# rwl/blu

Hardware: AMD Instinct MI355X
Metric: factorize nnz/s + achieved HBM GB/s, 100k x 100k 10-nnz/col basis (higher is better)
Workload: dtype f64

## Files before the change

### blu_amd/csrc/blu_dev.h

```cpp
#pragma once
#include <hip/hip_runtime.h>
#include <stdint.h>
#include <hip/hip_cooperative_groups.h>
#include <rocprim/warp/warp_reduce.hpp>
#include <rocprim/warp/warp_scan.hpp>

#define BLU_WAVE 64

#ifndef BLU_DYN_SHARED
#define BLU_DYN_SHARED(T, name, bytes) extern __shared__ __attribute__((aligned(16))) T name[]
#endif
#ifdef BLU_PROFILE_FILLS
#define FILL_STAMP_BEGIN() long long fill_t0_ = (long long)__builtin_amdgcn_s_memtime()
#define FILL_STAMP(S, k)                                                 \
    do {                                                                 \
        if (threadIdx.x == 0) {                                          \
            const long long t_ = (long long)__builtin_amdgcn_s_memtime(); \
            (S)->prof[k] += t_ - fill_t0_;                               \
            fill_t0_ = t_;                                               \
        }                                                                \
    } while (0)
#else
#define FILL_STAMP_BEGIN() \
    do {                   \
    } while (0)
#define FILL_STAMP(S, k) \
    do {                 \
    } while (0)
#endif
#ifdef BLU_EMU_BUILD
#define BLU_WAVES_PER_EU(lo, hi)
#else
#define BLU_WAVES_PER_EU(lo, hi) __attribute__((amdgpu_waves_per_eu(lo, hi)))
#endif

enum {
    ST_RUNNING = 0,
    ST_DONE = 1,
    ST_STOPPED = 2,
    ST_NEED_L = 3,
    ST_NEED_U = 4,
    ST_NEED_CW = 5,
    ST_NEED_RW = 6,
    ST_INVALID_ARG = 7,
    ST_ERROR = 8
};

struct Scalars {
    int status;
    int err_line;
    int rank;
    int rankdef;
    int rank0;
    int min_colnz;
    int min_rownz;
    int pivot_row;
    int pivot_col;
    int bump_size;
    int cused, rused;
    int lused, uused;
    int need;
    int l_nz, u_nz;
    int fill_paths;
    long long matrix_nz;
    long long bump_nz;
    long long nsearch_pivot;
    long long factor_flops;
    long long nexpand;
    long long ngarbage;
    long long d3_hits;
    long long npivot_kind[6];
    long long nfast[4];
    long long nrun[4];
    double min_pivot, max_pivot;
    double onenorm, infnorm;
    double norm_l, norm_u, normest_l_inv, normest_u_inv, condest_l, condest_u, residual_test;
    long long prof[48];
    long long prof2[14];
};

#define DEVLU_SCALARS(X)                                                                               \
    X(int, m)                                                                                          \
    X(int, nzbias)                                                                      \
    X(int, maxsearch)                                                                                  \
    X(int, pad)                                                                                        \
    X(int, search_rows)                                                                                \
    X(int, no_fast)                    \
    X(int, skip_stats)              \
    X(double, droptol)                                                                                 \
    X(double, abstol)                                                                                  \
    X(double, reltol)                                                                                  \
    X(double, stretch)                                                                                 \
    X(long long, b_i_len)                                                                              \
    X(int, nzcap)                                                                                      \
    X(int, carena_cap)                                                                                 \
    X(int, rarena_cap)                                                                                 \
    X(int, lcap)                                                                                       \
    X(int, ucap)

#define DEVLU_ARRAYS_HOT(X)                                                                            \
    X(int, pinv) X(int, qinv) X(int, prow) X(int, pcol)                                                \
    X(LineRec, crec) X(LineRec, rrec) X(HeadRec, chead) X(HeadRec, rhead)                              \
    X(int, cidx) X(double, cval) X(int, ridx)                                                          \
    X(int, lbeg) X(int, ubeg) X(int, lidx) X(int, uidx) X(double, lval) X(double, uval)
#define DEVLU_ARRAYS_COLD(X)                                                                           \
    X(const unsigned long long, b_begin) X(const unsigned long long, b_end) X(const unsigned long long, b_i) \
    X(const double, b_x)                                                                               \
    X(int, bc_ptr) X(int, bc_idx) X(double, bc_val) X(int, bt_ptr) X(int, bt_idx) X(double, bt_val)    \
    X(int, rowmark) X(int, colmark) X(int, tnew) X(int, tnewr) X(double, txrj)                         \
    X(unsigned long long, tmask) X(double, gwork) X(int, iw0) X(int, iw1) X(int, iw2)
#define DEVLU_ARRAYS(X) DEVLU_ARRAYS_HOT(X) DEVLU_ARRAYS_COLD(X)

struct __attribute__((aligned(32))) LineRec {
    int beg, len, cap;
    int flink, blink;
    int spare;
    double max;
};
struct __attribute__((aligned(8))) HeadRec {
    int flink, blink;
};
static_assert(sizeof(LineRec) == 32 && sizeof(HeadRec) == 8, "record layout");
#define LINEREC_BEG 0
#define LINEREC_LEN 4
#define LINEREC_CAP 8
#define LINEREC_FLINK 12
#define LINEREC_BLINK 16
#define LINEREC_MAX 24

struct DevLU {
#define X(T, n) T n;
// ... 477 lines not shown
```

### blu_amd/csrc/blu_hip.hip

```cpp
#include <hip/hip_runtime.h>

#include <algorithm>
#include <cmath>
#include <cstdio>
#include <cstdlib>
#include <cstring>
#include <string>
#include <vector>

#include "../../include/blu_hip.h"
#include "blu_dev.h"
#include "k_finish.hip"
#define BLU_NS pv_single
#define BLU_CFG_WAVE 0
#include "k_pivot.hip"
#undef BLU_NS
#undef BLU_CFG_WAVE
#define BLU_NS pv_wave
#define BLU_CFG_WAVE 1
#include "k_pivot.hip"
#undef BLU_NS
#undef BLU_CFG_WAVE
#define BLU_NS pv_wave2
#define BLU_CFG_WAVE 2
// ... 473 lines not shown
    case BLU_STAT_TIME_FACTORIZE: return h->t_total;
    case BLU_STAT_TIME_SINGLETONS: return h->t_phase[0];
    case BLU_STAT_TIME_SEARCH_PIVOT: {
        double tot = 0.0;
        for (int k = 0; k < 4; k++) tot += (double)s.prof[k];
        return tot > 0.0 ? h->t_pivot * (double)s.prof[0] / tot : 0.0;
    }
    case BLU_STAT_TIME_ELIM_PIVOT: {
        double tot = 0.0;
        for (int k = 0; k < 4; k++) tot += (double)s.prof[k];
        return tot > 0.0 ? h->t_pivot * (1.0 - (double)s.prof[0] / tot) : h->t_pivot;
    }
    case BLU_STAT_UPDATE_COST_DENOM: return h->update_cost_denom;
    case BLU_STAT_RANKDEF: return (double)s.rankdef;
    case BLU_STAT_L_MEM: return (double)h->D.lcap;
    case BLU_STAT_U_MEM: return (double)h->D.ucap;
    case BLU_STAT_W_MEM: return (double)h->D.carena_cap + (double)h->D.rarena_cap;
    case BLU_STAT_L_FLOPS: return (double)h->sp_l_flops;
    case BLU_STAT_U_FLOPS: return (double)h->sp_u_flops;
    case BLU_STAT_NFORREST: return h->upd_for_nfact == h->nfactorize ? (double)h->ust.nforrest : 0.0;
    case BLU_STAT_PIVOT_ERROR: return h->upd_for_nfact == h->nfactorize ? h->ust.pivot_error : 0.0;
    case BLU_STAT_R_NZ: return h->upd_for_nfact == h->nfactorize ? (double)h->ust.r_nz : 0.0;
    case BLU_STAT_R_FLOPS: return h->upd_for_nfact == h->nfactorize ? (double)h->ust.r_flops : 0.0;
    case BLU_STAT_MAX_ETA: return h->upd_for_nfact == h->nfactorize ? h->ust.max_eta : 0.0;
    case BLU_STAT_NSYMPERM_TOTAL: return (double)h->ust.nsymperm_total;
    case BLU_STAT_NFORREST_TOTAL: return (double)h->ust.nforrest_total;
    case BLU_STAT_DEV_NUNSYMPERM_TOTAL: return (double)h->ust.nunsymperm_total;
    case BLU_STAT_UPDATE_COST:
        return (h->upd_for_nfact == h->nfactorize ? h->ust.update_cost_numer : 0.0) / blu_hip_get_stat(h, BLU_STAT_UPDATE_COST_DENOM);
    case 44: case 45: case 46: case 47: return h->t_phase[key - 44];
    case 108: case 109: return h->t_phase[key - 108 + 4];
    case 43: return (double)h->sp_branch;
    case BLU_STAT_DEV_TIME_PIVOT_LOOP: return h->t_pivot;
    case BLU_STAT_DEV_TIME_TOTAL: return h->t_total;
    case BLU_STAT_DEV_RELAUNCHES: return (double)h->relaunches;
    case 50: return (double)s.d3_hits;
    case 51: return (double)s.npivot_kind[0];
    case 52: return (double)s.npivot_kind[1];
    case 53: return (double)s.npivot_kind[2];
    case 54: return (double)s.npivot_kind[3];
    case 55: return (double)s.npivot_kind[4];
    case 56: return (double)s.npivot_kind[5];
    case 110: case 111: case 116: case 117: return (double)s.nfast[key < 116 ? key - 110 : key - 114];
    case 112: return (double)s.cused;
    case 113: return (double)s.rused;
    case 114: return (double)h->D.carena_cap;
    case 115: return (double)h->D.lcap;
    case 120: return (double)h->last_pivot_regs;
    case 118: return (double)h->last_pivot_kernel;
    case 119: return (double)s.fill_paths;
    case 121: case 122: return (double)s.nrun[key - 121];
    case 123: return (double)s.nrun[2];
    case 125: return (double)s.nrun[3];
    case 126: return (double)h->chain_defects;
    case 131: case 132: case 133: case 134: case 135: case 136: case 137: case 138: case 139: case 140: case 141: case 142: case 143: case 144:
        return (double)s.prof2[key - 131];
    case 57: return (double)s.err_line;
    case 58: return (double)s.status;
    case 60: case 61: case 62: case 63: case 64: case 65: case 66: case 67: case 68: case 69: case 70: case 71: case 72: case 73: case 74: case 75:
    case 76: case 77: case 78: case 79: case 80: case 81: case 82: case 83:
    case 84: case 85: case 86: case 87: case 88: case 89: case 90: case 91:
    case 92: case 93: case 94: case 95: case 96: case 97: case 98: case 99: case 100: case 101: case 102: case 103: case 104: case 105: case 106: case 107:
        return (double)s.prof[key - 60];
    default: return NAN;
    }
}

extern "C" const char *blu_hip_last_error(const blu_hip *h) { return h ? h->err.c_str() : "null handle"; }
extern "C" const char *blu_hip_version(void)
{
#if defined(BLU_EWCHECK)
    return "blu_hip 0.2 (gfx950; self-checking build: early / speculative searches verified in the kernel)";
#elif defined(BLU_PROFILE)
    return "blu_hip 0.2 (gfx950; phase-timing build)";
#else
    return "blu_hip 0.2 (gfx950)";
#endif
}
extern "C" int blu_hip_device_count(void)
{
    int n = 0;
    if (hipGetDeviceCount(&n) != hipSuccess) return 0;
    return n;
}

static bool ensure_gwork(blu_hip *h, int cols)
{
    if (cols <= h->gwork_cols) return true;
    DevLU &D = h->D;
    const size_t n = (size_t)cols * ((size_t)h->m + 1);
    dfree(D.gwork);
    h->gwork_cols = 0;
    if (!dalloc(h, &D.gwork, n) || !hip_ok(h, hipMemset(D.gwork, 0, n * sizeof(double)), "hipMemset")) return false;
    h->gwork_cols = cols;
    return true;
}
static int64_t grown(blu_hip *h, int64_t cap, int64_t need_extra)
{
    const double f = std::max(1.0, h->realloc_factor);
    int64_t n = (int64_t)((double)(cap + need_extra) * f) + 64;
    return std::min<int64_t>(n, kIntMax);
}
static bool grow_l(blu_hip *h, int need)
{
    DevLU &D = h->D;
    const int64_t n = grown(h, D.lcap, need);
    if (n <= D.lcap) { h->err = "L storage limit (2^31 entries) reached"; return false; }
    if (!dgrow(h, &D.lidx, (size_t)h->hs.lused, (size_t)n) || !dgrow(h, &D.lval, (size_t)h->hs.lused, (size_t)n)) return false;
// ... 597 lines not shown
```

### blu_amd/csrc/k_pivot.hip

```cpp
#include "blu_dev.h"

namespace BLU_NS {

__shared__ int g_pivot_err;
__shared__ int g_pivot_err_line;
#undef DEV_CHECK
#define DEV_CHECK(S, cond)                               \
    do {                                                 \
        if (!(cond)) {                                   \
            set_error((S), ST_ERROR, __LINE__);          \
            g_pivot_err = 1;                             \
        }                                                \
    } while (0)

#if BLU_CFG_WAVE
#include "k_pivot_wave_types.h"
#else
#include "k_pivot_fast_types.h"
#endif

#ifdef BLU_PROFILE
__shared__ long long g_pstamp[56];
#define PROF_STAMP(k)                                                      \
    do {                                                                   \
        if (threadIdx.x == 0) g_pstamp[k] = (long long)__builtin_amdgcn_s_memtime(); \
    } while (0)
#define PROF_STAMP_L0(k)                                                           \
    do {                                                                           \
        if (lane_id() == 0) g_pstamp[k] = (long long)__builtin_amdgcn_s_memtime(); \
    } while (0)
#define PROF_WAIT() asm volatile("s_waitcnt vmcnt(0)" ::: "memory")
#else
#define PROF_STAMP(k) \
    do {              \
    } while (0)
#define PROF_STAMP_L0(k) \
    do {                 \
    } while (0)
#define PROF_WAIT() \
    do {            \
    } while (0)
#endif

struct alignas(16) Sm {
    Fast fa;
    struct alignas(16) {
        int pr, pc, exit_code, head_exit;
    };
    struct alignas(16) {
        int nzc, nzr, pcb, prb;
    };
#ifdef BLU_PROFILE
    long long prof[48];
    long long prof2[14];
#else
    long long prof[1];
#endif
#if !BLU_CFG_WAVE
    Fast fb;
    struct alignas(16) {
        int nx_pr, nx_pc, nx_nzr, nx_where;
    };
    struct alignas(16) {
        int nx_nzc, nx_kind, nx_pcb, nx_prb;
    };
    int nx_nsr, nx_minc;
    int nx_whole;
    int mg;
    long long nrun[4];
#endif
    int rank, rankdef, min_colnz, min_rownz;
    int cused, rused, lused, uused;
    int need;
    int flag_small;
    int other_row, where, ncancel, nfill;
    int stop_at, need_search;
    double pivot, other_value;
    long long nsearch, flops, nexpand, d3;
    long long kinds[6];
    long long nfast[4];
    int sh[40];
    long long shl[20];
#if BLU_CFG_WAVE
    unsigned long long wmax[BLU_CFG_WAVE];
#else
    unsigned long long wmax[16];
#endif
#if BLU_CFG_WAVE
    double swork[WV_WCAP];
#else
    double swork[16 * 64];
#endif
};

__device__ __forceinline__ void list_remove1(const LinkF &flink, const LinkB &blink, int e)
{
    const int f = flink[e], b = blink[e];
    flink[b] = f;
    blink[f] = b;
    flink[e] = e;
    blink[e] = e;
}
__device__ __forceinline__ void list_add1(int e, int list, const LinkF &flink, const LinkB &blink, int nelem)
{
    const int t = blink[nelem + list];
    blink[nelem + list] = e;
    blink[e] = t;
    flink[t] = e;
    flink[e] = nelem + list;
}

__device__ __forceinline__ int wave_list_move_batch(const LinkF &flink, const LinkB &blink, int nelem, gcint_p elems, gcint_p keys, int n,
                                                    gint_p mark, int big)
{
    const int lane = lane_id();
    int minkey = big;
    for (int c0 = 0; c0 < n; c0 += 64) {
        const int q = c0 + lane;
        if (q < n && keys[q] >= 0) mark[elems[q]] = 1;
    }
    wave_mem_sync();
    for (int c0 = 0; c0 < n; c0 += 64) {
// ... 982 lines not shown
    if (pc < 0 || pr < 0) return;
    sm->pcb = D.cbeg[pc];
    sm->prb = D.rbeg[pr];
    sm->nzc = D.clen[pc];
    sm->nzr = D.rlen[pr];
    sm->flag_small = 0;
    sm->ncancel = 0;
    DEV_CHECK(S, D.pinv[pr] == -1 && D.qinv[pc] == -1);
    DEV_CHECK(S, sm->nzc >= 1 && sm->nzr >= 1);
    if (sm->lused + (sm->nzc - 1) > D.lcap) {
        sm->exit_code = ST_NEED_L;
        sm->need = sm->nzc - 1;
    } else if (sm->uused + (sm->nzr - 1) > D.ucap) {
        sm->exit_code = ST_NEED_U;
        sm->need = sm->nzr - 1;
    }
}

#if BLU_CFG_WAVE
#include "k_pivot_wave.hip"
#else
__device__ __forceinline__ void pivot_loop_body(DevLU *Ds, int stop_at, Sm *sm, Mc *mc)
{
    const DevGP D(&Ds[blockIdx.x]);
    Scalars *S = D.s;
    const int tid = threadIdx.x, w = wave_id(), lane = lane_id();
    const int m = D.m;

    if (S->status != ST_RUNNING) return;
    if (tid == 0) {
        sm->rank = S->rank;
        sm->rankdef = S->rankdef;
        sm->min_colnz = S->min_colnz;
        sm->min_rownz = S->min_rownz;
        sm->cused = S->cused;
        sm->rused = S->rused;
        sm->lused = S->lused;
        sm->uused = S->uused;
        sm->pr = S->pivot_row;
        sm->pc = S->pivot_col;
        sm->exit_code = 0;
        sm->need = 0;
        sm->nsearch = 0;
        sm->flops = 0;
        sm->nexpand = 0;
        sm->d3 = 0;
        sm->stop_at = stop_at;
        sm->fa.kind = 0;
        sm->fa.ewValid = 0;
        sm->fa.spOk = 0;
        for (int k = 0; k < 6; k++) sm->kinds[k] = 0;
        sm->mg = 0;
        sm->nrun[0] = sm->nrun[1] = sm->nrun[2] = sm->nrun[3] = 0;
#ifdef BLU_PROFILE
        for (int k = 0; k < 48; k++) sm->prof[k] = 0;
        for (int k = 0; k < 14; k++) sm->prof2[k] = 0;
        for (int k = 0; k < 56; k++) g_pstamp[k] = 0;
#endif
    }
    for (int k = tid; k < (int)blockDim.x; k += blockDim.x) sm->swork[k] = 0.0;
    if (tid < 16) sm->wmax[tid] = 0ull;
    for (int k = tid; k < 2 * KGMAX; k += blockDim.x) sm->fa.kg[0][k] = 0ull;
    if (tid == 0) {
        g_pivot_err = 0;
        g_pivot_err_line = 0;
    }
    mc_reset(D, mc, tid, (int)blockDim.x);
    __syncthreads();

#ifdef BLU_PROFILE
#define PROF_ADD(k, a, b)                                                                                           \
    do {                                                                                                            \
        const long long d_ = g_pstamp[a] - g_pstamp[b];                                                             \
        if (g_pstamp[b] >= g_pstamp[0] && d_ >= 0 && d_ < (1LL << 28)) sm->prof[k] += d_;                            \
    } while (0)
#define PROF_ADD2(k, a, b)                                                                                          \
    do {                                                                                                            \
        const long long d_ = g_pstamp[a] - g_pstamp[b];                                                             \
        if (g_pstamp[b] >= g_pstamp[0] && d_ >= 0 && d_ < (1LL << 28)) sm->prof2[k] += d_;                           \
    } while (0)
    auto prof_account = [&](int kind_done, int nzc_done, int nzr_done) {
        {
            const int kk = kind_done == 1 ? 1 : (kind_done == 2 ? 2 : 3);
            PROF_ADD(0, 1, 0);
            PROF_ADD(kk, 2, 1);
            sm->prof[3 + kk] += 1;
            if (kk == 1) {
                const int by = g_pstamp[1] == g_pstamp[0] ? 8 : 11;
                PROF_ADD2(by, 2, 0);
                PROF_ADD2(by + 1, 2, 3);
                sm->prof2[by + 2] += 1;
                PROF_ADD(7, 3, 1);
                PROF_ADD(22, 6, 3);
                PROF_ADD(23, 24, 3);
                PROF_ADD(24, 25, 3);
                PROF_ADD(25, 26, 25);
                PROF_ADD(26, 27, 26);
                PROF_ADD(27, 28, 27);
                PROF_ADD(30, 30, 27);
                PROF_ADD(31, 31, 30);
                PROF_ADD(28, 29, 28);
                PROF_ADD(29, 2, 29);
                sm->prof[32] += nzr_done - 1;
                sm->prof[33] += nzc_done - 1;
                PROF_ADD(34, 33, 1);
                PROF_ADD(35, 34, 33);
                PROF_ADD(36, 35, 34);
                PROF_ADD(37, 36, 35);
                PROF_ADD(38, 37, 36);
                PROF_ADD(39, 38, 37);
                PROF_ADD(40, 3, 38);
                if (g_pstamp[44] > g_pstamp[1]) {
                    PROF_ADD(41, 41, 1);
                    PROF_ADD(42, 42, 41);
                    PROF_ADD(43, 43, 42);
                    PROF_ADD(44, 44, 43);
                    sm->prof[45] += 1;
                }
                if (g_pstamp[46] > g_pstamp[3]) {
                    PROF_ADD(46, 45, 3);
                    PROF_ADD(47, 46, 3);
                    sm->prof2[7] += 1;
                }
            }
            if (kk == 2) {
                PROF_ADD2(0, 1, 0);
                PROF_ADD2(1, 49, 48);
                PROF_ADD2(2, 50, 48);
                PROF_ADD2(3, 51, 48);
                PROF_ADD2(4, 2, 48);
                PROF_ADD2(5, 48, 1);
            }
            if (kk != 3) {
                PROF_ADD(8, 8, 0);
                PROF_ADD(9, 9, 8);
                PROF_ADD(10, 10, 9);
                PROF_ADD(11, 11, 10);
                PROF_ADD(12, 12, 11);
                PROF_ADD(13, 13, 12);
                PROF_ADD(14, 14, 13);
                PROF_ADD(15, 1, 14);
                if (g_pstamp[16] > g_pstamp[8]) {
                    PROF_ADD(16, 17, 16);
                    PROF_ADD(17, 18, 17);
                    PROF_ADD(18, 10, 18);
                    PROF_ADD(19, 19, 8);
                    PROF_ADD(20, 20, 19);
                    sm->prof[21] += 1;
                }
            }
        }
    };
#endif
    long long ew_mcb = 0;
    int ew_fb = 0;
    for (;;) {
        if (w == 0) {
            if (lane == 0) {
                if (g_pivot_err) sm->exit_code = ST_ERROR;
                else if (sm->rank + sm->rankdef >= m) sm->exit_code = ST_DONE;
                else if (sm->stop_at >= 0 && sm->pc < 0 && sm->rank + sm->rankdef >= sm->stop_at) sm->exit_code = ST_STOPPED;
                sm->need_search = sm->pc < 0;
                sm->head_exit = sm->exit_code;
            }
            wave_mem_sync();
            const bool heads_stale = mc->dirty;
            WAVE_LOCKSTEP();
            if (heads_stale) {
                mc_reset(D, mc, lane, 64);
                wave_mem_sync();
            }
            PROF_STAMP(0);
            if (!sm->head_exit) {
                bool handled = false;
                if (sm->need_search) {
// ... 91 lines not shown
        } else {
            if (tid == 0) mc->dirty = 1;
            if (nz_row == 1) ok = pivot_singleton_row(D, sm);
            else if (nz_col == 1) ok = pivot_singleton_col(D, sm);
            else if (nz_col == 2) ok = pivot_doubleton_col(D, sm);
            else ok = pivot_general(D, sm, nz_col - 1 <= 64);
        }
        if (!ok) break;
        PROF_STAMP(2);
#ifdef BLU_PROFILE
        if (tid == 0) prof_account(kind, nz_col, nz_row);
#endif

        if (tid == 0) {
            const int rank = sm->rank;
            if (sm->flag_small && nz_row > 1) {
                for (int pos = D.ubeg[rank]; pos < D.ubeg[rank + 1]; pos++) {
                    const int j = D.uidx[pos];
                    if (D.colmax[j] == 0.0 || D.colmax[j] < D.abstol) {
                        remove_col_serial(D, sm, j);
                        mc->dirty = 1;
                    }
                }
            }
            sm->flops += (long long)(nz_col - 1) * (long long)(nz_row - 1);
            D.pinv[pr] = rank;
            D.qinv[pc] = rank;
            D.prow[rank] = pr;
            D.pcol[rank] = pc;
            sm->pc = -1;
            sm->pr = -1;
            sm->rank = rank + 1;
        }
    }

    if (tid == 0) {
        S->rank = sm->rank;
        S->rankdef = sm->rankdef;
        S->min_colnz = sm->min_colnz;
        S->min_rownz = sm->min_rownz;
        S->cused = sm->cused;
        S->rused = sm->rused;
        S->lused = sm->lused;
        S->uused = sm->uused;
        S->pivot_row = sm->pr;
        S->pivot_col = sm->pc;
        S->need = sm->need;
        S->nsearch_pivot += sm->nsearch;
        S->factor_flops += sm->flops;
        S->nexpand += sm->nexpand;
        S->d3_hits += sm->d3;
        for (int k = 0; k < 6; k++) S->npivot_kind[k] += sm->kinds[k];
        for (int k = 0; k < 4; k++) S->nrun[k] += sm->nrun[k];
#ifdef BLU_PROFILE
        for (int k = 0; k < 48; k++) S->prof[k] += sm->prof[k];
        for (int k = 0; k < 14; k++) S->prof2[k] += sm->prof2[k];
#endif
        if (sm->exit_code == ST_ERROR && g_pivot_err_line) set_error(S, ST_ERROR, g_pivot_err_line);
        if (S->status == ST_RUNNING) S->status = sm->exit_code;
    }
}

__global__ void __launch_bounds__(1024) k_pivot_loop(DevLU *Ds, int stop_at)
{
    __shared__ Sm smem;
    __shared__ Mc mcache;
    pivot_loop_body(Ds, stop_at, &smem, &mcache);
}
#endif

}
#undef PROF_STAMP
#undef PROF_STAMP_L0
#undef PROF_WAIT
#undef COLD
#undef DEV_CHECK
#define DEV_CHECK(S, cond)                                   \
    do {                                                     \
        if (!(cond)) set_error((S), ST_ERROR, __LINE__);     \
    } while (0)
```

### blu_amd/csrc/k_pivot_fast.hip

```cpp

__device__ __forceinline__ unsigned hslot(int k, int bits) { return ((unsigned)k * 2654435761u) >> (32 - bits); }
__device__ __forceinline__ void probe_overrun(int line)
{
    g_pivot_err = 1;
    g_pivot_err_line = line;
}
__device__ __forceinline__ void hrow_insert(Fast *f, int k, int v)
{
    unsigned s = hslot(k, HROW_BITS);
    const unsigned long long want = ((unsigned long long)(unsigned)k << 32) | (unsigned)v;
    for (int n = 0; n < HROW; n++) {
        const unsigned long long old = atomicCAS(&f->hRow[s], ~0ull, want);
        if (old == ~0ull || (int)(old >> 32) == k) return;
        s = (s + 1) & (HROW - 1);
    }
    probe_overrun(__LINE__);
}
__device__ __forceinline__ int hrow_lookup(const Fast *f, int k)
{
    unsigned s = hslot(k, HROW_BITS);
    for (int n = 0; n < HROW; n++) {
        const unsigned long long x = f->hRow[s];
        if ((int)(x >> 32) == k) return (int)(x & 0xffffffffull);
        if (x == ~0ull) return 0;
// ... 1404 lines not shown
    while (ncand < K && nz <= m && !bad) {
        const int k = nz + lane;
        const int h = k <= m ? LC.fl(m + k) : m + k;
        unsigned long long ne = __ballot(k <= m && h != m + k);
        while (ne && ncand < K && !bad) {
            const int b = __ffsll((long long)ne) - 1;
            ne &= ne - 1;
            int j = wave_bcast_i(h, b);
            const int znz = nz + b;
            int guard = 0;
            while (j < m && ncand < K) {
                const int fl = D.cflink.el(j), cb = D.cbeg[j], cl = D.clen[j];
                const double cmx = D.colmax[j];
                if (cl != znz || cmx == 0.0 || !(cmx >= D.abstol) || ++guard > m + 2) {
                    bad = true;
                    break;
                }
                if (lane == 0) {
                    fa->cJ[ncand] = j;
                    fa->cNz[ncand] = znz;
                    fa->cB[ncand] = cb;
                    fa->cL[ncand] = cl;
                    fa->cMx[ncand] = cmx;
                    fa->cOff[ncand] = total;
                }
                total += cl;
                ncand++;
                lastnz = znz;
                j = fl;
            }
        }
        nz += 64;
    }
    if (bad || ncand < K || total > STGMAX) return;
    SPEC_STAT(1);
    if (lane == 0) {
        fa->cOff[ncand] = total;
        fa->ncand = ncand;
        fa->spLastNz = lastnz;
        fa->spOk = 1;
    }
    wave_mem_sync();
    PROF_STAMP_L0(42);
}

__device__ __forceinline__ bool spec_cond(const Sm *sm, const Fast *cs, const int *keys, int n)
{
    const int lane = lane_id();
    if (!sm->fa.spOk || sm->flag_small || cs->anycancel || n >= 64) return false;
    const int kq = lane < n ? keys[lane] : 0x7fffffff;
    return __ballot(kq <= 0) == 0ull;
}

__device__ __forceinline__ void spec_finish(const DevGP &D, Sm *sm, const Fast *cs, int n)
{
    const int lane = lane_id();
    Fast *fa = &sm->fa;
    const int ncand = fa->ncand;
    {
        const int lastnz = fa->spLastNz;
        const int key = lane < n ? cs->tNew[1 + lane] : 0x7fffffff;
        const unsigned long long inb = __ballot(key < lastnz);
        if (inb) {
            int uJ = 0, uNz = 0x7fffffff, uB = 0, uL = 0;
            double uMx = 0.0;
            if (lane < ncand) {
                uJ = fa->cJ[lane];
                uNz = fa->cNz[lane];
                uB = fa->cB[lane];
                uL = fa->cL[lane];
                uMx = fa->cMx[lane];
            }
            int ule = 0;
            for (int i = 0; i < ncand; i++) ule += fa->cNz[i] <= key;
            int before = 0, below = 0;
            unsigned long long mb = inb;
            while (mb) {
                const int b = __ffsll((long long)mb) - 1;
                mb &= mb - 1;
                const int kb = __builtin_amdgcn_readlane(key, b);
                before += (kb < key) || (kb == key && b < lane);
                below += kb < uNz;
            }
            const int posM = ule + before, posU = lane + below;
            wave_mem_sync();
            if (lane < ncand && posU < ncand) {
                fa->cJ[posU] = uJ;
                fa->cNz[posU] = uNz;
                fa->cB[posU] = uB;
                fa->cL[posU] = uL;
                fa->cMx[posU] = uMx;
            }
            if (((inb >> lane) & 1ull) && posM < ncand) {
                fa->cJ[posM] = cs->tJ[1 + lane];
                fa->cNz[posM] = key;
                fa->cB[posM] = cs->tB[1 + lane];
                fa->cL[posM] = key;
                fa->cMx[posM] = cs->tMx[1 + lane];
            }
            wave_mem_sync();
            if (lane == 0) {
                int off = 0;
                for (int i = 0; i < ncand; i++) {
                    fa->cOff[i] = off;
                    off += fa->cL[i];
                }
                fa->cOff[ncand] = off;
            }
            wave_mem_sync();
            SPEC_STAT(4);
        }
    }
    const int total = fa->cOff[ncand];
    if (total > STGMAX) return;
    const int off1 = ncand > 1 ? fa->cOff[1] : 0x7fffffff, off2 = ncand > 2 ? fa->cOff[2] : 0x7fffffff,
              off3 = ncand > 3 ? fa->cOff[3] : 0x7fffffff;
    const long long BIG = 0x7fffffffffffffffLL;
    long long mcb = BIG;
    int fb = 0x7fffffff;
    for (int base = 0; base < total; base += 64) {
        const int f = base + lane;
        if (f < total) {
            const int c = (f >= off1) + (f >= off2) + (f >= off3);
            const int pos = fa->cB[c] + (f - fa->cOff[c]);
            const int idx = D.cidx[pos];
            const double val = D.cval[pos];
            const int rb = D.rbeg[idx], rl = D.rlen[idx], rc = D.rcap[idx];
            fa->sI[f] = idx;
            fa->sV[f] = val;
            fa->sB[f] = rb;
            fa->sL[f] = rl;
            fa->sC[f] = rc;
            const double tol = fmax(D.abstol, D.reltol * fa->cMx[c]);
            const double x = fabs(val);
            if (!(x == 0.0 || x < tol)) {
                const long long cost = (long long)(fa->cNz[c] - 1) * (long long)(rl - 1);
                if (cost < mcb) {
                    mcb = cost;
                    fb = f;
                }
            }
        }
    }
    PROF_WAIT();
    PROF_STAMP_L0(43);
    SPEC_STAT(2);
    const long long key = wave_min_ll(mcb != BIG ? mcb * 256LL + (long long)fb : BIG);
    if (key == BIG) return;
    SPEC_STAT(3);
    if (lane == 0) {
        fa->spKey = key;
        fa->ewNsr = ncand;
        fa->ewValid = 2;
    }
    wave_mem_sync();
    PROF_STAMP_L0(44);
}

__device__ __forceinline__ bool scol_setup_next(const DevGP &D, Sm *sm, Mc *mc, Fast *nxt, int rl_cur);
__device__ __forceinline__ bool small_setup_next(const DevGP &D, Sm *sm, Mc *mc, Fast *nxt, int cnz1_cur, int rnz1_cur);
__device__ __forceinline__ void fast_small(const DevGP &D, Sm *sm, Mc *mc, Fast *fa, int pr, int pc, int nzc, int nzr, long long &ew_mcb, int &ew_fb)
{
    const int w = wave_id(), nw = num_waves(), lane = lane_id();
    const int m = D.m;
    const int cnz1 = nzc - 1, rnz1 = nzr - 1;
    const double pivot = fa->pcV[0];
    DEV_CHECK(D.s, pivot != 0.0);

    double *work = &sm->swork[w * 64];
    const int ntask = rnz1 + cnz1;
    PROF_STAMP(4);
    const bool split = nw >= 8 && rnz1 < 64;
    const int nwt = split ? nw - 1 : nw;
    const LinksC LC{D, mc};
    const bool early = split && !D.search_rows;
    if (split && w == nw - 1) {
        if (early) __builtin_amdgcn_s_setprio(3);
        const bool lnk = fa->tLnk != 0;
        wave_list_unlink_set(LC, fa->tJ + 1, rnz1, -1, InHCol{fa, 1, 0}, pc, lnk ? fa->tFl + 1 : nullptr, lnk ? fa->tBl + 1 : nullptr, -1);
        if (early) {
            wave_mem_sync();
            spec_walk(D, sm, mc);
            __builtin_amdgcn_s_setprio(0);
        }
    }
    for (int base = 0; base < ntask && w < nwt; base += 3 * nwt) {
        int li[3], tt[3];
        double lv[3];
        tt[0] = base + w;
        tt[1] = base + 2 * nwt - 1 - w;
        tt[2] = base + 2 * nwt + w;
        int lb[3], ll[3];
        bool isc[3];
#pragma unroll
        for (int u = 0; u < 3; u++) {
            const int t = tt[u];
            isc[u] = t < rnz1;
            const bool isr = !isc[u] && t < ntask;
            const int q = isc[u] ? t + 1 : 0, p = isr ? t - rnz1 + 1 : 0;
            const int cb_ = fa->tB[q], cl_ = fa->tL[q], rb_ = fa->prB[p], rl_ = fa->prL[p];
            lb[u] = isc[u] ? cb_ : rb_;
            ll[u] = isc[u] ? cl_ : (isr ? rl_ : 0);
        }
#pragma unroll
        for (int u = 0; u < 3; u++) {
            li[u] = -1;
            lv[u] = 0.0;
            if (lane < ll[u]) {
                if (isc[u]) {
                    li[u] = D.cidx[lb[u] + lane];
                    lv[u] = D.cval[lb[u] + lane];
                } else {
                    li[u] = D.ridx[lb[u] + lane];
                }
            }
        }
#ifdef BLU_PROFILE
        if (w == 1 && base == 0) {
            PROF_STAMP_L0(33);
            PROF_WAIT();
            PROF_STAMP_L0(34);
        }
#endif
#pragma unroll
        for (int u = 0; u < 3; u++) {
            const int t = tt[u];
            if (t < rnz1) {
                if (ll[u] <= 64) fast_col_short(D, sm, mc, fa, t + 1, work, li[u], lv[u], pr, cnz1, pivot);
                else fast_col(D, sm, mc, fa, t + 1, work, li[u], lv[u], pr, cnz1, pivot);
            } else if (t < ntask) {
                if (ll[u] <= 64) fast_row_short(D, sm, fa, t - rnz1 + 1, li[u], pc, rnz1);
                else fast_row(D, sm, fa, t - rnz1 + 1, li[u], pc, rnz1);
            }
#ifdef BLU_PROFILE
            if (w == 1 && base == 0) PROF_STAMP_L0(35 + u);
#endif
        }
    }
#ifdef BLU_PROFILE
    if (w == 1) {
        PROF_WAIT();
        PROF_STAMP_L0(38);
    }
#endif
    PROF_STAMP(5);
    __syncthreads();
    PROF_STAMP(3);
    if (fa->anycancel) {
        for (int p = 1 + w; p <= cnz1; p += nw) fast_fixrow(D, fa, p, rnz1);
        __syncthreads();
    }
    const bool spec = early && (w == 0 || w == nw - 1) && spec_cond(sm, fa, fa->tNew + 1, rnz1);
    Fast *other = fa == &sm->fa ? &sm->fb : &sm->fa;
    if (w == 0 && !spec) {
        bool merged = false;
        if (early) {
            early_search(D, sm, mc, fa, fa->tJ + 1, fa->tNew + 1, fa->tB + 1, fa->tMx + 1, rnz1, 1, ew_mcb, ew_fb);
            merged = scol_setup_next(D, sm, mc, other, rnz1 + 1);
        }
        if (lane == 0) sm->mg = merged ? 1 : 0;
    }
    if (w == nw - 1 && spec) {
        spec_finish(D, sm, fa, rnz1);
        PROF_STAMP_L0(45);
        const bool merged = small_setup_next(D, sm, mc, other, cnz1, rnz1);
        if (lane == 0) sm->mg = merged ? 1 : 0;
        PROF_STAMP_L0(46);
    }
    if (w == (early ? 3 : 0)) {
        fast_write_u(D, sm, fa, 1, rnz1, -1);
        if (lane == 0) {
            D.colmax[pc] = fa->pcV[0];
            D.clen[pc] = 0;
            D.rlen[pr] = 0;
            sm->kinds[3]++;
        }
        PROF_STAMP_L0(6);
    }
    if (w == 1 % nw) {
        fast_write_l(D, sm, fa, cnz1);
        PROF_STAMP_L0(24);
    }
    if (w == 2 % nw) {
        PROF_STAMP_L0(25);
        const int mn = split ? wave_list_append_set(LC, m, fa->tJ + 1, fa->tNew + 1, rnz1, m + 2, sm->fa.kg[0], mc->pFl + 1)
                             : wave_list_move_batch_set(LC, m, fa->tJ + 1, fa->tNew + 1, rnz1, InHCol{fa, 1, 0}, m + 2, pc, sm->fa.kg[0]);
        if (lane == 0 && mn < sm->min_colnz) sm->min_colnz = mn;
        if (lane == 0) {
            mc->prevValid = split && fa == &sm->fa ? 1 : 0;
            mc->prevBase = 1;
        }
        PROF_WAIT();
        PROF_STAMP_L0(29);
    }
    if (D.search_rows && w == 3 % nw) {
        if (lane == 0) list_remove1(D.rflink, D.rblink, pr);
        wave_mem_sync();
        const int mn = wave_list_move_batch_set(LinksG{D.rflink, D.rblink}, m, fa->pcI + 1, fa->rNew + 1, cnz1, InHRow{fa}, m + 2, -1, sm->fa.kg[1]);
        if (lane == 0 && mn < sm->min_rownz) sm->min_rownz = mn;
    }
    __syncthreads();
}

__device__ __forceinline__ bool scol_setup_next(const DevGP &D, Sm *sm, Mc *mc, Fast *nxt, int rl_cur)
{
    const int lane = lane_id();
    Fast *st = &sm->fa;
    if (st->ewValid != 1) return false;
    if (g_pivot_err || mc->dirty) return false;
    const int nrd = sm->rank + 1 + sm->rankdef;
    if (nrd >= D.m || (sm->stop_at >= 0 && nrd >= sm->stop_at)) return false;
    const int pc = st->cJ[0], pr = st->sI[0], prb = st->sB[0], nzr = st->sL[0];
    if (nzr < 2 || nzr >= 64) return false;
    if (sm->lused > D.lcap || (long long)sm->uused + (rl_cur - 1) + (nzr - 1) > (long long)D.ucap) return false;
    const int jq0 = lane < nzr ? D.ridx[prb + lane] : -1;
    for (int s = lane; s < HCOL; s += 64) nxt->hCol[s] = ~0ull;
    const unsigned long long hb = __ballot(jq0 == pc);
    if (!hb) return false;
    const int wpos = __ffsll((long long)hb) - 1;
    if (lane < nzr) {
        const int tb = D.cbeg[jq0], tl = D.clen[jq0], tc = D.ccap[jq0];
        nxt->tJ[lane] = jq0;
        nxt->tB[lane] = tb;
        nxt->tL[lane] = tl;
        nxt->tC[lane] = tc;
        hcol_insert(nxt, jq0, lane);
    }
    if (lane == 0) {
        nxt->pcI[0] = pr;
        nxt->pcV[0] = st->sV[0];
        nxt->prB[0] = prb;
        nxt->prL[0] = nzr;
        nxt->prC[0] = st->sC[0];
        nxt->kind = 2;
        nxt->where = wpos;
        nxt->anycancel = 0;
        nxt->tLnk = 0;
        sm->nx_pr = pr;
        sm->nx_pc = pc;
        sm->nx_nzr = nzr;
        sm->nx_where = wpos;
        sm->nx_nzc = 1;
        sm->nx_kind = 2;
        sm->nx_prb = prb;
        sm->nx_pcb = st->cB[0];
        sm->nx_nsr = st->ewNsr;
        sm->nx_minc = 1;
        sm->nx_whole = 0;
        st->ewValid = 0;
    }
    return true;
}

__device__ __forceinline__ bool small_setup_next(const DevGP &D, Sm *sm, Mc *mc, Fast *nxt, int cnz1_cur, int rnz1_cur)
{
    const int lane = lane_id();
    Fast *st = &sm->fa;
    if (st->ewValid != 2) return false;
    if (g_pivot_err || mc->dirty) return false;
    const int nrd = sm->rank + 1 + sm->rankdef;
    if (nrd >= D.m || (sm->stop_at >= 0 && nrd >= sm->stop_at)) return false;
    const int ncand = st->ncand;
    const int off1 = ncand > 1 ? st->cOff[1] : 0x7fffffff, off2 = ncand > 2 ? st->cOff[2] : 0x7fffffff,
              off3 = ncand > 3 ? st->cOff[3] : 0x7fffffff;
    const int fsel = (int)(st->spKey & 255LL);
    const int csel = (fsel >= off1) + (fsel >= off2) + (fsel >= off3);
    const int coff = st->cOff[csel];
    const int pc = st->cJ[csel], pr = st->sI[fsel];
    const int nzc = st->cL[csel], pcb = st->cB[csel], where = fsel - coff;
    const int nzr = st->sL[fsel], prb = st->sB[fsel];
    int kind = 0;
    if (nzr >= 2 && nzr <= 64) {
        if (nzc == 1) kind = 2;
        else if (nzc >= 3 && nzc <= 64) kind = 1;
    }
    if (kind == 0) return false;
    if ((long long)sm->lused + cnz1_cur + (nzc - 1) > (long long)D.lcap || (long long)sm->uused + rnz1_cur + (nzr - 1) > (long long)D.ucap) return false;
    const int jq0 = lane < nzr ? D.ridx[prb + lane] : -1;
    if (kind == 1) {
        for (int s = lane; s < HROW; s += 64) nxt->hRow[s] = ~0ull;
    }
    for (int s = lane; s < HCOL; s += 64) nxt->hCol[s] = ~0ull;
    int hr_idx0 = 0, hr_slot0 = 0, hr_len0 = 0;
    if (lane < nzc) {
        const int slot = (lane == where) ? 0 : (lane == 0 ? where : lane);
        const int idx = st->sI[coff + lane], rlv = st->sL[coff + lane];
        nxt->pcI[slot] = idx;
        nxt->pcV[slot] = st->sV[coff + lane];
        nxt->prB[slot] = st->sB[coff + lane];
        nxt->prL[slot] = rlv;
        nxt->prC[slot] = st->sC[coff + lane];
        hr_slot0 = slot;
        hr_idx0 = idx;
        hr_len0 = rlv;
    }
    const unsigned long long hb = __ballot(jq0 == pc);
    if (!hb) return false;
    const int wpos = __ffsll((long long)hb) - 1;
    int tb = 0, tl = 0, tc = 0;
    if (lane < nzr) {
        tb = D.cbeg[jq0];
        tl = D.clen[jq0];
        tc = D.ccap[jq0];
    }
    int gc = 0, gr = 0;
    if (kind == 1 && hr_slot0 >= 1) {
        hrow_insert(nxt, hr_idx0, hr_slot0);
        const int n = hr_len0 + nzr - 1;
        gr = n + stretch_of(D.stretch, n) + D.pad;
    }
    if (lane < nzr) {
        const int slot = kind == 1 ? ((lane == wpos) ? 0 : (lane == 0 ? wpos : lane)) : lane;
        nxt->tJ[slot] = jq0;
        nxt->tB[slot] = tb;
        nxt->tL[slot] = tl;
        nxt->tC[slot] = tc;
        hcol_insert(nxt, jq0, slot);
        if (kind == 1 && lane != wpos) {
            const int n = tl + nzc - 1;
            gc = n + stretch_of(D.stretch, n) + D.pad;
        }
    }
    if (kind == 1) {
        const long long both = wave_sum_ll(((long long)gc << 32) | (long long)(unsigned)gr);
        if ((long long)sm->cused + (both >> 32) > (long long)D.carena_cap || (long long)sm->rused + (both & 0xffffffffLL) > (long long)D.rarena_cap)
            return false;
    }
    if (lane == 0) {
        nxt->kind = kind;
        nxt->where = wpos;
        nxt->anycancel = 0;
        nxt->tLnk = 0;
        sm->nx_pr = pr;
        sm->nx_pc = pc;
        sm->nx_nzr = nzr;
        sm->nx_where = wpos;
        sm->nx_nzc = nzc;
        sm->nx_kind = kind;
        sm->nx_prb = prb;
        sm->nx_pcb = pcb;
        sm->nx_nsr = st->ewNsr;
        sm->nx_minc = st->cNz[0];
        sm->nx_whole = 1;
        st->ewValid = 0;
    }
    return true;
}

#ifdef BLU_EWCHECK
__device__ __forceinline__ void scol_setup_check(const DevGP &D, Sm *sm, Mc *mc, Fast *nxt)
{
    const int lane = lane_id();
    Fast *T = nxt;
    Fast *R = &sm->fa;
    if (nxt == R) {
        T = &sm->fb;
        T->tJ[lane] = R->tJ[lane];
        T->tB[lane] = R->tB[lane];
        T->tL[lane] = R->tL[lane];
        T->tC[lane] = R->tC[lane];
        for (int s = lane; s < HCOL; s += 64) T->hCol[s] = R->hCol[s];
        if (lane == 0) {
            T->kind = R->kind;
            T->where = R->where;
            T->pcI[0] = R->pcI[0];
            T->pcV[0] = R->pcV[0];
        }
    }
    wave_mem_sync();
    const int o_pr = sm->pr, o_pc = sm->pc, o_pcb = sm->pcb, o_prb = sm->prb, o_nzc = sm->nzc, o_nzr = sm->nzr;
    const int o_exit = sm->exit_code, o_need = sm->need, o_minc = sm->min_colnz;
    const long long o_ns = sm->nsearch;
    wave_mem_sync();
    int nsr2 = 0;
    bool okc = mk_express(D, sm, mc, nsr2);
    if (okc) {
        mk_pick(D, sm, 0, 0, nsr2, true);
        wave_mem_sync();
        const int n = sm->nx_nzr;
        okc = sm->pr == sm->nx_pr && sm->pc == sm->nx_pc && sm->nzr == n && sm->nzc == 1 && sm->prb == sm->nx_prb && sm->pcb == sm->nx_pcb &&
              nsr2 == sm->nx_nsr && sm->exit_code == o_exit && sm->min_colnz == o_minc && R->kind == 2 && T->kind == 2 && R->where == T->where &&
              R->pcI[0] == T->pcI[0] && R->pcV[0] == T->pcV[0];
        if (okc && lane < n) {
            const int j = T->tJ[lane];
            okc = R->tJ[lane] == j && R->tB[lane] == T->tB[lane] && R->tL[lane] == T->tL[lane] && R->tC[lane] == T->tC[lane] &&
                  hcol_slot(R, j) == lane && hcol_slot(T, j) == lane;
        }
        int cntR = 0, cntT = 0;
        for (int s = lane; s < HCOL; s += 64) {
            cntR += __popcll(__ballot(R->hCol[s] != ~0ull));
            cntT += __popcll(__ballot(T->hCol[s] != ~0ull));
        }
        okc = okc && cntR == n && cntT == n;
    }
    wave_mem_sync();
    if (lane == 0) {
        sm->pr = o_pr;
        sm->pc = o_pc;
        sm->pcb = o_pcb;
// ... 245 lines not shown
```

### blu_amd/keys.py

```python
OK = 0
REALLOCATE = 1
WARNING_SINGULAR_MATRIX = 2
ERROR_INVALID_CALL = -2
ERROR_ARGUMENT_MISSING = -3
ERROR_INVALID_ARGUMENT = -4
ERROR_MAXIMUM_UPDATES = -5
ERROR_SINGULAR_UPDATE = -6
ERROR_OUT_OF_MEMORY = -9
ERROR_DEVICE = -100

PARAM_DROPTOL = 0
PARAM_ABSTOL = 1
PARAM_RELTOL = 2
PARAM_NZBIAS = 3
PARAM_MAXSEARCH = 4
PARAM_PAD = 5
PARAM_STRETCH = 6
PARAM_COMPRESS_THRES = 7
PARAM_SPARSE_THRES = 8
PARAM_SEARCH_ROWS = 9
PARAM_REALLOC_FACTOR = 10

STAT_M = 0
STAT_NUPDATE = 1
STAT_NFACTORIZE = 2
STAT_L_NZ = 3
STAT_U_NZ = 4
STAT_MIN_PIVOT = 5
STAT_MAX_PIVOT = 6
STAT_CONDEST_L = 7
STAT_CONDEST_U = 8
STAT_NORM_L = 9
STAT_NORM_U = 10
STAT_NORMEST_L_INV = 11
STAT_NORMEST_U_INV = 12
STAT_ONENORM = 13
STAT_INFNORM = 14
STAT_RESIDUAL_TEST = 15
STAT_MATRIX_NZ = 16
STAT_RANK = 17
STAT_BUMP_SIZE = 18
STAT_BUMP_NZ = 19
STAT_NSEARCH_PIVOT = 20
STAT_NEXPAND = 21
STAT_NGARBAGE = 22
STAT_FACTOR_FLOPS = 23
STAT_TIME_FACTORIZE = 24
STAT_TIME_SINGLETONS = 25
STAT_TIME_SEARCH_PIVOT = 26
STAT_TIME_ELIM_PIVOT = 27
STAT_UPDATE_COST_DENOM = 28
STAT_RANKDEF = 29
STAT_L_MEM = 30
STAT_U_MEM = 31
STAT_W_MEM = 32
STAT_L_FLOPS = 33
STAT_U_FLOPS = 34
STAT_NFORREST = 35
STAT_PIVOT_ERROR = 36
STAT_R_NZ = 37
STAT_R_FLOPS = 38
STAT_MAX_ETA = 39
STAT_DEV_TIME_PIVOT_LOOP = 40
STAT_DEV_TIME_TOTAL = 41
STAT_DEV_RELAUNCHES = 42
STAT_NSYMPERM_TOTAL = 48
STAT_NFORREST_TOTAL = 49
STAT_DEV_NUNSYMPERM_TOTAL = 59
STAT_UPDATE_COST = 124
```

Baseline: 1.441 million.

## Split speculative next-pivot setup across two waves with LDS handshake

```diff
diff --git a/blu_amd/csrc/blu_dev.h b/blu_amd/csrc/blu_dev.h
--- a/blu_amd/csrc/blu_dev.h
+++ b/blu_amd/csrc/blu_dev.h
@@ -72,11 +72,12 @@
     long long npivot_kind[6];
     long long nfast[4];
     long long nrun[4];
+    long long nsplit[2];
     double min_pivot, max_pivot;
     double onenorm, infnorm;
     double norm_l, norm_u, normest_l_inv, normest_u_inv, condest_l, condest_u, residual_test;
     long long prof[48];
-    long long prof2[14];
+    long long prof2[20];
 };
 
 #define DEVLU_SCALARS(X)                                                                               \
diff --git a/blu_amd/csrc/blu_hip.hip b/blu_amd/csrc/blu_hip.hip
--- a/blu_amd/csrc/blu_hip.hip
+++ b/blu_amd/csrc/blu_hip.hip
@@ -549,8 +549,10 @@
     case 121: case 122: return (double)s.nrun[key - 121];
     case 123: return (double)s.nrun[2];
     case 125: return (double)s.nrun[3];
+    case 127: case 128: return (double)s.nsplit[key - 127];
     case 126: return (double)h->chain_defects;
     case 131: case 132: case 133: case 134: case 135: case 136: case 137: case 138: case 139: case 140: case 141: case 142: case 143: case 144:
+    case 145: case 146: case 147: case 148: case 149: case 150:
         return (double)s.prof2[key - 131];
     case 57: return (double)s.err_line;
     case 58: return (double)s.status;
diff --git a/blu_amd/csrc/k_pivot.hip b/blu_amd/csrc/k_pivot.hip
--- a/blu_amd/csrc/k_pivot.hip
+++ b/blu_amd/csrc/k_pivot.hip
@@ -20,7 +20,7 @@
 #endif
 
 #ifdef BLU_PROFILE
-__shared__ long long g_pstamp[56];
+__shared__ long long g_pstamp[64];
 #define PROF_STAMP(k)                                                      \
     do {                                                                   \
         if (threadIdx.x == 0) g_pstamp[k] = (long long)__builtin_amdgcn_s_memtime(); \
@@ -52,7 +52,7 @@
     };
 #ifdef BLU_PROFILE
     long long prof[48];
-    long long prof2[14];
+    long long prof2[20];
 #else
     long long prof[1];
 #endif
@@ -68,6 +68,10 @@
     int nx_whole;
     int mg;
     long long nrun[4];
+    volatile int hs_go;
+    volatile int hs_done;
+    long long hs_gr;
+    long long nsplit[2];
 #endif
     int rank, rankdef, min_colnz, min_rownz;
     int cused, rused, lused, uused;
@@ -1156,10 +1160,14 @@
         for (int k = 0; k < 6; k++) sm->kinds[k] = 0;
         sm->mg = 0;
         sm->nrun[0] = sm->nrun[1] = sm->nrun[2] = sm->nrun[3] = 0;
+        sm->nsplit[0] = sm->nsplit[1] = 0;
+        sm->hs_go = 0;
+        sm->hs_done = 0;
+        sm->hs_gr = 0;
 #ifdef BLU_PROFILE
         for (int k = 0; k < 48; k++) sm->prof[k] = 0;
-        for (int k = 0; k < 14; k++) sm->prof2[k] = 0;
-        for (int k = 0; k < 56; k++) g_pstamp[k] = 0;
+        for (int k = 0; k < 20; k++) sm->prof2[k] = 0;
+        for (int k = 0; k < 64; k++) g_pstamp[k] = 0;
 #endif
     }
     for (int k = tid; k < (int)blockDim.x; k += blockDim.x) sm->swork[k] = 0.0;
@@ -1225,6 +1233,12 @@
                     PROF_ADD(46, 45, 3);
                     PROF_ADD(47, 46, 3);
                     sm->prof2[7] += 1;
+                    PROF_ADD2(14, 52, 3);
+                    PROF_ADD2(15, 53, 3);
+                    PROF_ADD2(16, 54, 3);
+                    PROF_ADD2(17, 55, 3);
+                    PROF_ADD2(18, 56, 3);
+                    PROF_ADD2(19, 57, 3);
                 }
             }
             if (kk == 2) {
@@ -1422,9 +1436,10 @@
         S->d3_hits += sm->d3;
         for (int k = 0; k < 6; k++) S->npivot_kind[k] += sm->kinds[k];
         for (int k = 0; k < 4; k++) S->nrun[k] += sm->nrun[k];
+        for (int k = 0; k < 2; k++) S->nsplit[k] += sm->nsplit[k];
 #ifdef BLU_PROFILE
         for (int k = 0; k < 48; k++) S->prof[k] += sm->prof[k];
-        for (int k = 0; k < 14; k++) S->prof2[k] += sm->prof2[k];
+        for (int k = 0; k < 20; k++) S->prof2[k] += sm->prof2[k];
 #endif
         if (sm->exit_code == ST_ERROR && g_pivot_err_line) set_error(S, ST_ERROR, g_pivot_err_line);
         if (S->status == ST_RUNNING) S->status = sm->exit_code;
diff --git a/blu_amd/csrc/k_pivot_fast.hip b/blu_amd/csrc/k_pivot_fast.hip
--- a/blu_amd/csrc/k_pivot_fast.hip
+++ b/blu_amd/csrc/k_pivot_fast.hip
@@ -1480,11 +1480,17 @@
     return __ballot(kq <= 0) == 0ull;
 }
 
-__device__ __forceinline__ void spec_finish(const DevGP &D, Sm *sm, const Fast *cs, int n)
+struct SpecWin {
+    long long key;
+    int csel, coff;
+    int pr, nzr, prb;
+};
+__device__ __forceinline__ void spec_finish(const DevGP &D, Sm *sm, const Fast *cs, int n, SpecWin &win)
 {
     const int lane = lane_id();
     Fast *fa = &sm->fa;
     const int ncand = fa->ncand;
+    win.key = -1;
     {
         const int lastnz = fa->spLastNz;
         const int key = lane < n ? cs->tNew[1 + lane] : 0x7fffffff;
@@ -1539,13 +1545,14 @@
             SPEC_STAT(4);
         }
     }
+    PROF_STAMP_L0(52);
     const int total = fa->cOff[ncand];
     if (total > STGMAX) return;
     const int off1 = ncand > 1 ? fa->cOff[1] : 0x7fffffff, off2 = ncand > 2 ? fa->cOff[2] : 0x7fffffff,
               off3 = ncand > 3 ? fa->cOff[3] : 0x7fffffff;
     const long long BIG = 0x7fffffffffffffffLL;
     long long mcb = BIG;
-    int fb = 0x7fffffff;
+    int fb = 0x7fffffff, bI = 0, bL = 0, bB = 0;
     for (int base = 0; base < total; base += 64) {
         const int f = base + lane;
         if (f < total) {
@@ -1553,7 +1560,15 @@
             const int pos = fa->cB[c] + (f - fa->cOff[c]);
             const int idx = D.cidx[pos];
             const double val = D.cval[pos];
+            if (base == 0) {
+                PROF_WAIT();
+                PROF_STAMP_L0(53);
+            }
             const int rb = D.rbeg[idx], rl = D.rlen[idx], rc = D.rcap[idx];
+            if (base == 0) {
+                PROF_WAIT();
+                PROF_STAMP_L0(54);
+            }
             fa->sI[f] = idx;
             fa->sV[f] = val;
             fa->sB[f] = rb;
@@ -1566,6 +1581,9 @@
                 if (cost < mcb) {
                     mcb = cost;
                     fb = f;
+                    bI = idx;
+                    bL = rl;
+                    bB = rb;
                 }
             }
         }
@@ -1576,17 +1594,40 @@
     const long long key = wave_min_ll(mcb != BIG ? mcb * 256LL + (long long)fb : BIG);
     if (key == BIG) return;
     SPEC_STAT(3);
-    if (lane == 0) {
-        fa->spKey = key;
-        fa->ewNsr = ncand;
-        fa->ewValid = 2;
-    }
-    wave_mem_sync();
+    const int fsel = (int)(key & 255LL);
+    const int wl = fsel & 63;
+    win.key = key;
+    win.csel = (fsel >= off1) + (fsel >= off2) + (fsel >= off3);
+    win.coff = win.csel == 0 ? 0 : (win.csel == 1 ? off1 : (win.csel == 2 ? off2 : off3));
+    win.pr = wave_bcast_i(bI, wl);
+    win.nzr = wave_bcast_i(bL, wl);
+    win.prb = wave_bcast_i(bB, wl);
     PROF_STAMP_L0(44);
 }
 
+#ifdef BLU_EMU_BUILD
+#define HS_LDS(T) T *
+#else
+#define HS_LDS(T) __attribute__((address_space(3))) T *
+#endif
+#define HS_SPIN 64
+#define HS_BOUND (1 << 20)
+__device__ __forceinline__ int hs_get(const volatile int *p) { return *(HS_LDS(const volatile int))p; }
+__device__ __forceinline__ void hs_put(volatile int *p, int v) { *(HS_LDS(volatile int))p = v; }
+__device__ __forceinline__ int hs_wait(const volatile int *p)
+{
+    int v = hs_get(p);
+    for (int it = 0; v == 0 && it < HS_BOUND; it++) {
+        if (it >= HS_SPIN) __builtin_amdgcn_s_sleep(1);
+        v = hs_get(p);
+    }
+    return v;
+}
+
+struct SpecWin;
 __device__ __forceinline__ bool scol_setup_next(const DevGP &D, Sm *sm, Mc *mc, Fast *nxt, int rl_cur);
-__device__ __forceinline__ bool small_setup_next(const DevGP &D, Sm *sm, Mc *mc, Fast *nxt, int cnz1_cur, int rnz1_cur);
+__device__ __forceinline__ bool small_setup_next(const DevGP &D, Sm *sm, Mc *mc, Fast *nxt, int cnz1_cur, int rnz1_cur, const SpecWin &win);
+__device__ __forceinline__ void small_setup_help(const DevGP &D, Sm *sm, Fast *nxt);
 __device__ __forceinline__ void fast_small(const DevGP &D, Sm *sm, Mc *mc, Fast *fa, int pr, int pc, int nzc, int nzr, long long &ew_mcb, int &ew_fb)
 {
     const int w = wave_id(), nw = num_waves(), lane = lane_id();
@@ -1671,6 +1712,10 @@
         PROF_STAMP_L0(38);
     }
 #endif
+    if (early && w == nwt - 1 && lane == 0) {
+        hs_put(&sm->hs_go, 0);
+        hs_put(&sm->hs_done, 0);
+    }
     PROF_STAMP(5);
     __syncthreads();
     PROF_STAMP(3);
@@ -1688,10 +1733,11 @@
         }
         if (lane == 0) sm->mg = merged ? 1 : 0;
     }
+    if (w == 0 && spec) small_setup_help(D, sm, other);
     if (w == nw - 1 && spec) {
-        spec_finish(D, sm, fa, rnz1);
-        PROF_STAMP_L0(45);
-        const bool merged = small_setup_next(D, sm, mc, other, cnz1, rnz1);
+        SpecWin win;
+        spec_finish(D, sm, fa, rnz1, win);
+        const bool merged = small_setup_next(D, sm, mc, other, cnz1, rnz1, win);
         if (lane == 0) sm->mg = merged ? 1 : 0;
         PROF_STAMP_L0(46);
     }
@@ -1780,48 +1826,43 @@
     return true;
 }
 
-__device__ __forceinline__ bool small_setup_next(const DevGP &D, Sm *sm, Mc *mc, Fast *nxt, int cnz1_cur, int rnz1_cur)
+__device__ __forceinline__ bool small_setup_next(const DevGP &D, Sm *sm, Mc *mc, Fast *nxt, int cnz1_cur, int rnz1_cur, const SpecWin &win)
 {
     const int lane = lane_id();
     Fast *st = &sm->fa;
-    if (st->ewValid != 2) return false;
-    if (g_pivot_err || mc->dirty) return false;
+    if (win.key < 0) {
+        if (lane == 0) hs_put(&sm->hs_go, 2);
+        return false;
+    }
+    const int ncand = st->ncand;
+    const int csel = win.csel, coff = win.coff;
+    const int pc = st->cJ[csel], nzc = st->cL[csel], pcb = st->cB[csel], minc = st->cNz[0];
+    const int pr = win.pr, nzr = win.nzr, prb = win.prb;
+    const int where = (int)(win.key & 255LL) - coff;
+    bool go = !(g_pivot_err || mc->dirty);
     const int nrd = sm->rank + 1 + sm->rankdef;
-    if (nrd >= D.m || (sm->stop_at >= 0 && nrd >= sm->stop_at)) return false;
-    const int ncand = st->ncand;
-    const int off1 = ncand > 1 ? st->cOff[1] : 0x7fffffff, off2 = ncand > 2 ? st->cOff[2] : 0x7fffffff,
-              off3 = ncand > 3 ? st->cOff[3] : 0x7fffffff;
-    const int fsel = (int)(st->spKey & 255LL);
-    const int csel = (fsel >= off1) + (fsel >= off2) + (fsel >= off3);
-    const int coff = st->cOff[csel];
-    const int pc = st->cJ[csel], pr = st->sI[fsel];
-    const int nzc = st->cL[csel], pcb = st->cB[csel], where = fsel - coff;
-    const int nzr = st->sL[fsel], prb = st->sB[fsel];
+    if (nrd >= D.m || (sm->stop_at >= 0 && nrd >= sm->stop_at)) go = false;
     int kind = 0;
     if (nzr >= 2 && nzr <= 64) {
         if (nzc == 1) kind = 2;
         else if (nzc >= 3 && nzc <= 64) kind = 1;
     }
-    if (kind == 0) return false;
-    if ((long long)sm->lused + cnz1_cur + (nzc - 1) > (long long)D.lcap || (long long)sm->uused + rnz1_cur + (nzr - 1) > (long long)D.ucap) return false;
-    const int jq0 = lane < nzr ? D.ridx[prb + lane] : -1;
-    if (kind == 1) {
-        for (int s = lane; s < HROW; s += 64) nxt->hRow[s] = ~0ull;
-    }
+    if (kind == 0) go = false;
+    if ((long long)sm->lused + cnz1_cur + (nzc - 1) > (long long)D.lcap || (long long)sm->uused + rnz1_cur + (nzr - 1) > (long long)D.ucap) go = false;
+    PROF_STAMP_L0(55);
+    const int jq0 = go && lane < nzr ? D.ridx[prb + lane] : -1;
+    if (lane == 0) {
+        st->spKey = win.key;
+        st->ewNsr = ncand;
+        st->ewValid = 2;
+    }
+    __builtin_amdgcn_fence(__ATOMIC_RELEASE, "workgroup");
+    if (lane == 0) hs_put(&sm->hs_go, go ? 1 : 2);
+    PROF_STAMP_L0(45);
+    if (!go) return false;
     for (int s = lane; s < HCOL; s += 64) nxt->hCol[s] = ~0ull;
-    int hr_idx0 = 0, hr_slot0 = 0, hr_len0 = 0;
-    if (lane < nzc) {
-        const int slot = (lane == where) ? 0 : (lane == 0 ? where : lane);
-        const int idx = st->sI[coff + lane], rlv = st->sL[coff + lane];
-        nxt->pcI[slot] = idx;
-        nxt->pcV[slot] = st->sV[coff + lane];
-        nxt->prB[slot] = st->sB[coff + lane];
-        nxt->prL[slot] = rlv;
-        nxt->prC[slot] = st->sC[coff + lane];
-        hr_slot0 = slot;
-        hr_idx0 = idx;
-        hr_len0 = rlv;
-    }
+    PROF_WAIT();
+    PROF_STAMP_L0(56);
     const unsigned long long hb = __ballot(jq0 == pc);
     if (!hb) return false;
     const int wpos = __ffsll((long long)hb) - 1;
@@ -1831,12 +1872,9 @@
         tl = D.clen[jq0];
         tc = D.ccap[jq0];
     }
-    int gc = 0, gr = 0;
-    if (kind == 1 && hr_slot0 >= 1) {
-        hrow_insert(nxt, hr_idx0, hr_slot0);
-        const int n = hr_len0 + nzr - 1;
-        gr = n + stretch_of(D.stretch, n) + D.pad;
-    }
+    PROF_WAIT();
+    PROF_STAMP_L0(57);
+    int gc = 0;
     if (lane < nzr) {
         const int slot = kind == 1 ? ((lane == wpos) ? 0 : (lane == 0 ? wpos : lane)) : lane;
         nxt->tJ[slot] = jq0;
@@ -1849,9 +1887,16 @@
             gc = n + stretch_of(D.stretch, n) + D.pad;
         }
     }
+    long long gcs = 0;
+    if (kind == 1) gcs = wave_sum_ll((long long)gc);
+    const int dn = hs_wait(&sm->hs_done);
+    __builtin_amdgcn_fence(__ATOMIC_ACQUIRE, "workgroup");
+    if (dn != 1) {
+        if (dn == 0 && lane == 0) atomicAdd((unsigned long long *)&sm->nsplit[1], 1ull);
+        return false;
+    }
     if (kind == 1) {
-        const long long both = wave_sum_ll(((long long)gc << 32) | (long long)(unsigned)gr);
-        if ((long long)sm->cused + (both >> 32) > (long long)D.carena_cap || (long long)sm->rused + (both & 0xffffffffLL) > (long long)D.rarena_cap)
+        if ((long long)sm->cused + gcs > (long long)D.carena_cap || (long long)sm->rused + sm->hs_gr > (long long)D.rarena_cap)
             return false;
     }
     if (lane == 0) {
@@ -1867,12 +1912,56 @@
         sm->nx_kind = kind;
         sm->nx_prb = prb;
         sm->nx_pcb = pcb;
-        sm->nx_nsr = st->ewNsr;
-        sm->nx_minc = st->cNz[0];
+        sm->nx_nsr = ncand;
+        sm->nx_minc = minc;
         sm->nx_whole = 1;
         st->ewValid = 0;
+        if (kind == 1) sm->nsplit[0]++;
     }
     return true;
+}
+
+__device__ __forceinline__ void small_setup_help(const DevGP &D, Sm *sm, Fast *nxt)
+{
+    const int lane = lane_id();
+    Fast *st = &sm->fa;
+    for (int s = lane; s < HROW; s += 64) nxt->hRow[s] = ~0ull;
+    const int go = hs_wait(&sm->hs_go);
+    __builtin_amdgcn_fence(__ATOMIC_ACQUIRE, "workgroup");
+    if (go != 1) {
+        if (go == 0 && lane == 0) {
+            hs_put(&sm->hs_done, 2);
+            atomicAdd((unsigned long long *)&sm->nsplit[1], 1ull);
+        }
+        return;
+    }
+    const int ncand = st->ncand;
+    const int off1 = ncand > 1 ? st->cOff[1] : 0x7fffffff, off2 = ncand > 2 ? st->cOff[2] : 0x7fffffff,
+              off3 = ncand > 3 ? st->cOff[3] : 0x7fffffff;
+    const int fsel = (int)(st->spKey & 255LL);
+    const int csel = (fsel >= off1) + (fsel >= off2) + (fsel >= off3);
+    const int coff = st->cOff[csel];
+    const int nzc = st->cL[csel], where = fsel - coff;
+    const int nzr = st->sL[fsel];
+    int gr = 0;
+    if (lane < nzc) {
+        const int slot = (lane == where) ? 0 : (lane == 0 ? where : lane);
+        const int idx = st->sI[coff + lane], rlv = st->sL[coff + lane];
+        nxt->pcI[slot] = idx;
+        nxt->pcV[slot] = st->sV[coff + lane];
+        nxt->prB[slot] = st->sB[coff + lane];
+        nxt->prL[slot] = rlv;
+        nxt->prC[slot] = st->sC[coff + lane];
+        if (nzc >= 3 && slot >= 1) {
+            hrow_insert(nxt, idx, slot);
+            const int n = rlv + nzr - 1;
+            gr = n + stretch_of(D.stretch, n) + D.pad;
+        }
+    }
+    const long long grs = wave_sum_ll((long long)gr);
+    if (lane == 0) sm->hs_gr = grs;
+    __builtin_amdgcn_fence(__ATOMIC_RELEASE, "workgroup");
+    if (lane == 0) hs_put(&sm->hs_done, 1);
 }
 
 #ifdef BLU_EWCHECK
diff --git a/blu_amd/keys.py b/blu_amd/keys.py
--- a/blu_amd/keys.py
+++ b/blu_amd/keys.py
@@ -68,3 +68,5 @@
 STAT_NFORREST_TOTAL = 49
 STAT_DEV_NUNSYMPERM_TOTAL = 59
 STAT_UPDATE_COST = 124
+DEVSTAT_SETUP_TWO_WAVES = 127
+DEVSTAT_SETUP_ABANDONED = 128
```

New measurement: 1.470 million, median of 6. +2.0%, better.
